# cule/multimot_track

Hardware: AMD Instinct MI355X
Metric: KITTI RGB-D frames/sec (ego+object poses) at 1/2/4/8 GPUs; CPU ref fps (higher is better)
Workload: dtype u8

## Files before the change

### include/mmt.h

```cpp
#ifndef MMT_H
#define MMT_H

#include <stddef.h>
#include <stdint.h>

#ifdef __cplusplus
extern "C" {
#endif

#define MMT_OK 0
#define MMT_EINVAL (-22)
#define MMT_ENOMEM (-12)
#define MMT_ENOSPC (-28)
#define MMT_EDEVICE (-5)
#define MMT_ESTATE (-77)

#define MMT_MAX_OBJECTS 15

typedef struct mmt_config {
  int width, height;
  float fx, fy, cx, cy;
  float k1, k2, p1, p2, k3;
  float bf;
  float th_depth;
// ... 75 lines not shown
                   const float* flow_uv, const int32_t* mask, double timestamp,
                   mmt_frame_result* res, mmt_motion* objs, int objs_cap);

int mmt_track_rgbd_chunk(mmt_ctx* ctx, int nframes, const uint8_t* const* bgr,
                         const uint16_t* const* disp256, const float* const* flow_uv,
                         const int32_t* const* mask, mmt_frame_result* res, mmt_motion* objs,
                         int objs_cap);

void* mmt_host_alloc(mmt_ctx* ctx, size_t bytes);
void mmt_host_free(mmt_ctx* ctx, void* p);

int mmt_track_rgbd_chunk_device(mmt_ctx* ctx, int nframes, const uint8_t* d_bgr,
                                size_t bgr_pitch, const uint16_t* d_disp, size_t disp_pitch,
                                const float* d_flow, size_t flow_pitch, const int32_t* d_mask,
                                size_t mask_pitch, mmt_frame_result* res, mmt_motion* objs,
                                int objs_cap, void* stream);

typedef struct mmt_flow_problem {
  int n;
  const float* obs;
  const float* flow;
  const float* depth;
  float Tcw_last[16];
  float init[16];
  float rp_thres;
  double prior_info;
  int max_iters;
  int use_noise;
  float g0;
  float fx, fy, cx, cy;
} mmt_flow_problem;
int mmt_pose_flow_solve(mmt_ctx* ctx, const mmt_flow_problem* problem, float* pose_out,
                        int* stats_out );

typedef struct mmt_pose_opt_problem {
  int n;
  const float* Xw;
  const float* obs;
  const float* inv_sigma2;
  float Tcw[16];
  float fx, fy, cx, cy, bf;
} mmt_pose_opt_problem;
int mmt_pose_optimization(mmt_ctx* ctx, const mmt_pose_opt_problem* problem, float* pose_out,
                          uint8_t* outlier_out, int* n_inliers);

int mmt_pnp_ransac(mmt_ctx* ctx, const float* pts3, const float* pts2, int n, float fx,
                   float fy, float cx, float cy, int max_iters, double reproj, double confidence,
                   double* R_out, double* t_out, int* inliers_out, int* n_inliers,
                   int* iters_out );

typedef struct mmt_pnpsolver_problem {
  int n;
  const float* pts3;
  const float* pts2;
  const float* sigma2;
  float fx, fy, cx, cy;
  double probability;
  int min_inliers;
  int max_iterations;
  int min_set;
  float epsilon;
  float th2;
} mmt_pnpsolver_problem;

typedef struct mmt_pnpsolver_state {
  int iterations;
// ... 303 lines not shown
```

### multimot_track_amd/__init__.py

```python
import ctypes
import os

import numpy as np

_HERE = os.path.dirname(os.path.abspath(__file__))
LIB_PATH = os.environ.get("MMT_LIB_PATH") or os.path.join(_HERE, "libmmt.so")
_LIB = None

KP_DTYPE = np.dtype([("x", "<f4"), ("y", "<f4"), ("size", "<f4"), ("angle", "<f4"),
                     ("response", "<f4"), ("octave", "<i4"), ("class_id", "<i4")])


class MmtConfig(ctypes.Structure):
    _fields_ = [("width", ctypes.c_int), ("height", ctypes.c_int),
                ("fx", ctypes.c_float), ("fy", ctypes.c_float), ("cx", ctypes.c_float),
                ("cy", ctypes.c_float), ("k1", ctypes.c_float), ("k2", ctypes.c_float),
                ("p1", ctypes.c_float), ("p2", ctypes.c_float), ("k3", ctypes.c_float),
                ("bf", ctypes.c_float), ("th_depth", ctypes.c_float), ("rgb", ctypes.c_int),
                ("orb_nfeatures", ctypes.c_int), ("orb_scale_factor", ctypes.c_float),
                ("orb_nlevels", ctypes.c_int), ("orb_ini_th_fast", ctypes.c_int),
                ("orb_min_th_fast", ctypes.c_int), ("noise_seed", ctypes.c_uint32),
                ("device_id", ctypes.c_int), ("max_batch", ctypes.c_int),
                ("fps", ctypes.c_float)]

# ... 497 lines not shown
            flow.data_ptr(), pitch(flow), mask.data_ptr(), pitch(mask), res, objs, MAX_OBJECTS,
            ctypes.c_void_p(stream)))
        if not parse:
            return res, objs
        return [_frame_dict(res[i], objs[i * MAX_OBJECTS:(i + 1) * MAX_OBJECTS])
                for i in range(nf)]

    def profile_enable(self, on=True):
        self._check(lib().mmt_profile_enable(self._h, int(on)))

    def profile_read(self, reset=False):
        p = MmtProfile()
        self._check(lib().mmt_profile_read(self._h, ctypes.byref(p), int(reset)))
        return dict(orb_ms=p.orb_ms, orb_launches=p.orb_launches, orb_frames=p.orb_frames)

    def flow_solve(self, obs, flow, depth, tcw_last, init, rp_thres, prior_info, max_iters,
                   K, use_noise=False, g0=0.0):
        obs = np.ascontiguousarray(obs, np.float32)
        flow = np.ascontiguousarray(flow, np.float32)
        depth = np.ascontiguousarray(depth, np.float32)
        pr = MmtFlowProblem()
        pr.n = len(depth)
        pr.obs, pr.flow, pr.depth = obs.ctypes.data, flow.ctypes.data, depth.ctypes.data
        pr.Tcw_last[:] = np.asarray(tcw_last, np.float32).reshape(16).tolist()
        pr.init[:] = np.asarray(init, np.float32).reshape(16).tolist()
        pr.rp_thres, pr.prior_info, pr.max_iters = rp_thres, prior_info, max_iters
        pr.use_noise, pr.g0 = int(use_noise), g0
        pr.fx, pr.fy, pr.cx, pr.cy = K
        pose = np.zeros(16, np.float32)
        st = np.zeros(3, np.int32)
        self._check(lib().mmt_pose_flow_solve(self._h, ctypes.byref(pr), _p(pose), _p(st)))
        return int(st[2]), pose.reshape(4, 4), dict(iterations=int(st[0]), inliers=int(st[1]))

    def pose_optimization(self, Xw, obs, inv_sigma2, tcw, K, bf):
        Xw = np.ascontiguousarray(Xw, np.float32)
        obs = np.ascontiguousarray(obs, np.float32)
        s2 = np.ascontiguousarray(inv_sigma2, np.float32)
        n = len(Xw)
        pr = MmtPoseOptProblem()
        pr.n = n
        pr.Xw, pr.obs, pr.inv_sigma2 = Xw.ctypes.data, obs.ctypes.data, s2.ctypes.data
        pr.Tcw[:] = np.asarray(tcw, np.float32).reshape(16).tolist()
        pr.fx, pr.fy, pr.cx, pr.cy = K
        pr.bf = bf
        pose = np.zeros(16, np.float32)
        out = np.zeros(max(n, 1), np.uint8)
        ninl = ctypes.c_int(0)
        self._check(lib().mmt_pose_optimization(self._h, ctypes.byref(pr), _p(pose), _p(out),
                                                ctypes.byref(ninl)))
        return ninl.value, pose.reshape(4, 4), out[:n].astype(bool)

    @staticmethod
    def _match_frame(kps, desc, depth, tcw, keep):
        kps = np.ascontiguousarray(kps)
        desc = np.ascontiguousarray(desc, np.uint8) if desc is not None else None
        depth = np.ascontiguousarray(depth, np.float32)
        keep += [kps, desc, depth]
        fr = MmtMatchFrame()
        fr.n = len(kps)
        fr.kps = kps.ctypes.data
        fr.desc = desc.ctypes.data if desc is not None else None
        fr.depth = depth.ctypes.data
        fr.Tcw[:] = np.asarray(tcw, np.float32).reshape(16).tolist()
        return fr

    def frame_grid(self, kps, depth):
# ... 481 lines not shown
```

### multimot_track_amd/csrc/mmt_capi_probes.hip

```cpp

#include <hip/hip_runtime.h>

#include <cstdint>

#include <algorithm>
#include <cmath>
#include <cstring>
#include <vector>

#include "mmt_ctx.h"
#include "mmt_devbuf.h"
#include "mmt_mat4.h"
#include "mmt_match.h"
#include "mmt_pnp.h"
#include "mmt_sim3.h"
#include "mmt_sim3opt.h"
#include "mmt_track.h"

using mmt::ArgError;
using mmt::DevBuf;
using mmt::DeviceError;

struct ProbeStage : mmt::Stage {
  uint8_t* d = nullptr;
// ... 101 lines not shown

static void check_feature_vector(const mmt_feature_vector* v, int n, std::vector<uint8_t>* once,
                                 int max_node) {
  if (v->n_nodes < 0) throw ArgError("negative node count");
  if (v->n_nodes == 0) return;
  if (!v->node_id || !v->node_start || !v->feat) throw ArgError("null feature vector arrays");
  if (v->node_start[0] != 0) throw ArgError("node_start[0] != 0");
  for (int k = 0; k < v->n_nodes; k++) {
    if (k > 0 && !(v->node_id[k - 1] < v->node_id[k])) throw ArgError("node ids not ascending");
    const int a = v->node_start[k], b = v->node_start[k + 1];
    if (b < a) throw ArgError("node_start not monotone");
    if (b - a > max_node) throw ArgError("a vocabulary node holds more than 16384 frame features");
    for (int q = a; q < b; q++) {
      const int f = v->feat[q];
      if (f < 0 || f >= n) throw ArgError("feature index out of range");
      if (once) {
        if ((*once)[f]) throw ArgError("a frame feature is listed in two nodes");
        (*once)[f] = 1;
      }
    }
  }
}

static void check_sft_keyframe(const mmt_sft_keyframe* k) {
  if (k->n < 0 || k->n > mmt::kMaxMatchKeys) throw ArgError("bad keyframe size");
  if (k->n > 0 && (!k->kps || !k->desc || !k->uR || !k->has_mp))
    throw ArgError("null keyframe arrays");
  std::vector<uint8_t> once((size_t)std::max(k->n, 1), 0);
  check_feature_vector(&k->fv, k->n, &once, INT32_MAX);
}

extern "C" {

int mmt_pose_flow_solve(mmt_ctx* ctx, const mmt_flow_problem* pr, float* pose_out,
                        int* stats_out) {
  if (!ctx || !pr || !pose_out || !stats_out || pr->n < 0) return MMT_EINVAL;
  return guard(ctx, [&] {
    MMT_HIP(hipSetDevice(ctx->cfg.device_id));
    hipStream_t s = ctx->stream;
    const int n = pr->n, cap = std::max(n, 1);
    DevBuf<float2> obs(cap), flow(cap);
    DevBuf<float> depth(cap), pose(16);
    DevBuf<double> scratch(mmt::flow_scratch_doubles(cap));
    DevBuf<int> st(3);
    DevBuf<mmt::FlowSolveDesc> dd(1);
    const int groups = mmt::flow_split_groups(n);
    DevBuf<unsigned long long> gx(groups > 1 ? mmt::kFlowSplitGranules : 1);
    if (groups > 1)
      MMT_HIP(hipMemsetAsync(gx.p, 0, sizeof(unsigned long long) * mmt::kFlowSplitGranules, s));
    obs.up((const float2*)pr->obs, n, s);
    flow.up((const float2*)pr->flow, n, s);
    depth.up(pr->depth, n, s);
    mmt::FlowSolveDesc d;
    memset(&d, 0, sizeof(d));
    d.n = n;
    d.obs = obs.p;
    d.flow = flow.p;
    d.depth = depth.p;
    memcpy(d.Tcw_last, pr->Tcw_last, 64);
    memcpy(d.init, pr->init, 64);
    d.rp_thres = pr->rp_thres;
    d.use_noise = pr->use_noise;
    d.g0 = pr->g0;
    d.max_iters = pr->max_iters;
    d.prior_info = pr->prior_info;
    d.fx = pr->fx; d.fy = pr->fy; d.cx = pr->cx; d.cy = pr->cy;
    d.scratch = scratch.p;
    d.cap = cap;
    d.pose_out = pose.p;
    d.stats = st.p;
    d.gx = gx.p;
    d.gx_seq = 1;
    dd.up(&d, 1, s);
    pose.up(pr->init, 16, s);
    if (groups > 1)
      mmt::launch_flow_lm_split(dd.p, groups, s);
    else
      mmt::launch_flow_lm(dd.p, 1, n, s);
    pose.down(pose_out, 16, s);
    st.down(stats_out, 3, s);
    MMT_HIP(hipStreamSynchronize(s));
    if (stats_out[2] == 2)
      throw mmt::DeviceError("pose flow solve: the split solve's workgroups were not resident together");
  });
}

int mmt_pose_optimization(mmt_ctx* ctx, const mmt_pose_opt_problem* pr, float* pose_out,
                          uint8_t* outlier_out, int* n_inliers) {
  if (!ctx || !pr || !pose_out || !n_inliers || pr->n < 0 ||
      (pr->n > 0 && (!pr->Xw || !pr->obs || !pr->inv_sigma2 || !outlier_out)))
    return MMT_EINVAL;
  return guard(ctx, [&] {
    MMT_HIP(hipSetDevice(ctx->cfg.device_id));
    hipStream_t s = ctx->stream;
    const int n = pr->n, cap = std::max(n, 1);
    DevBuf<float> X(3 * (size_t)cap), ob(3 * (size_t)cap), s2(cap), pose(16);
    DevBuf<uint8_t> outl(cap);
    DevBuf<int> ninl(1), fsc(n > mmt::kPoseOptMaxEdges ? cap : 1);
    DevBuf<double> esc(n > mmt::kPoseOptMaxEdges ? 3 * (size_t)cap : 1);
    DevBuf<mmt::PoseOptDesc> dd(1);
    X.up(pr->Xw, 3 * (size_t)n, s);
    ob.up(pr->obs, 3 * (size_t)n, s);
    s2.up(pr->inv_sigma2, n, s);
    mmt::PoseOptDesc d;
    memset(&d, 0, sizeof(d));
    d.n = n;
    d.Xw = X.p;
    d.obs = ob.p;
    d.inv_sigma2 = s2.p;
    memcpy(d.Tcw, pr->Tcw, 64);
    d.fx = pr->fx; d.fy = pr->fy; d.cx = pr->cx; d.cy = pr->cy; d.bf = pr->bf;
    d.pose_out = pose.p;
    d.outlier = outl.p;
    d.n_inliers = ninl.p;
    d.e_scratch = esc.p;
    d.f_scratch = fsc.p;
    dd.up(&d, 1, s);
// ... 571 lines not shown
```

### multimot_track_amd/csrc/mmt_lm.hip

```cpp

#include <hip/hip_runtime.h>

#include <cfloat>
#include <cstdio>
#include <cstdlib>

#include <algorithm>

#include "mmt_devmath.h"
#include "mmt_internal.h"
#include "mmt_lmstep.h"
#include "mmt_track.h"

namespace mmt {

namespace {

constexpr double kInfo = 0.1;

struct LMItem {
  double X[3];
  double ob[2];
  double pr[2];
  double f[2];
// ... 579 lines not shown
#pragma unroll
    for (int cc = 0; cc < 3; cc++) Rwl[3 * r + cc] = D.Tcw_last[4 * cc + r];
#pragma unroll
  for (int r = 0; r < 3; r++) {
    double s = 0;
#pragma unroll
    for (int k = 0; k < 3; k++) s += (double)Rwl[3 * r + k] * (double)D.Tcw_last[4 * k + 3];
    twl[r] = (float)(-s);
  }
  auto init_item = [&](int i, LMItem& it) {
    const int s = D.idx ? D.idx[i] : i;
    const float2 ob = D.obs[s];
    float z = D.depth[s];
    if (D.use_noise) z = (float)((double)z + (double)D.g0 * ((double)(z * z) / (725 * 0.5) * 0.15));
    const double u = ob.x, v = ob.y, dz = z;
    const double Xc0 = (u - c.cx) * dz / c.fx, Xc1 = (v - c.cy) * dz / c.fy, Xc2 = dz;
    it.X[0] = (double)Rwl[0] * Xc0 + (double)Rwl[1] * Xc1 + (double)Rwl[2] * Xc2 + (double)twl[0];
    it.X[1] = (double)Rwl[3] * Xc0 + (double)Rwl[4] * Xc1 + (double)Rwl[5] * Xc2 + (double)twl[1];
    it.X[2] = (double)Rwl[6] * Xc0 + (double)Rwl[7] * Xc1 + (double)Rwl[8] * Xc2 + (double)twl[2];
    it.ob[0] = u;
    it.ob[1] = v;
    const float2 fl = D.flow[s];
    it.pr[0] = fl.x;
    it.pr[1] = fl.y;
    it.f[0] = fl.x;
    it.f[1] = fl.y;
    it.xl[0] = it.xl[1] = 0;
    it.e[0] = it.e[1] = 0;
  };
  LMItem R[IR];
  const int n_reg = IR * nt;
  constexpr bool kCacheB = true;
  double RB[12];
  DSE3 P = dse3_from_float(D.init);
  const double hin = kInfo + c.pinfo;
  double* row = tile_row(sm.tile);
  {
    double mh = 0;
#pragma unroll
    for (int k = 0; k < IR; k++) {
      const int i = tid + k * nt;
      if (i < N) {
        init_item(lo + i, R[k]);
        if (k == 0)
          linearise<true>(c, P, R[k], R[k].f[0], R[k].f[1], row, 0.0, R[k].e[0], R[k].e[1],
                          R[k].w, R[k].bl[0], R[k].bl[1], mh, kCacheB ? RB : nullptr);
        else
          linearise<false>(c, P, R[k], R[k].f[0], R[k].f[1], row, 0.0, R[k].e[0], R[k].e[1],
                           R[k].w, R[k].bl[0], R[k].bl[1], mh);
      }
    }
    for (int i = n_reg + tid; i < N; i += nt) {
      LMItem it;
      init_item(lo + i, it);
      linearise<false>(c, P, it, it.f[0], it.f[1], row, 0.0, it.e[0], it.e[1], it.w, it.bl[0],
                       it.bl[1], mh);
      item_store(G, cap, lo + i, it);
    }
    if (tid >= N)
      for (int q = 0; q < kSums; q++) row[q] = 0;
#pragma unroll
    for (int o = 32; o > 0; o >>= 1) mh = fmax(mh, __shfl_xor(mh, o, 64));
    if ((tid & 63) == 0) sm.mh[tid >> 6] = mh;
  }
  int pb = 0;
  double vc = block_sum_tile_lanes<kSums>(sm.tile, sm.part[pb], nw);
  pb ^= 1;
// ... 1047 lines not shown
```

### multimot_track_amd/csrc/mmt_map.h

```cpp
#pragma once
#include <hip/hip_runtime.h>

#include <cstdint>
#include <functional>
#include <set>
#include <utility>
#include <vector>

#include "mmt_ba.h"
#include "mmt_bow.h"
#include "mmt_internal.h"
#include "mmt_mapgraph.h"
#include "mmt_match.h"
#include "mmt_track.h"

namespace mmt {

struct MapCamH {
  int W = 0, H = 0;
  float fx = 0, fy = 0, cx = 0, cy = 0, invfx = 0, invfy = 0, bf = 0;
  float thDepth = 0;
  int maxFrames = 0;
  int nlevels = 0;
  float logScale = 0;
// ... 22 lines not shown
  long n_lm = 0;
};

struct BowStatsH {
  long n_bow_frames = 0, n_trk = 0, n_trk_ok = 0, n_reloc = 0, n_reloc_ok = 0, n_reloc_cands = 0,
       n_pnp_found = 0, n_sbp_rounds = 0, n_triangulated = 0, n_sft_matches = 0, n_kfdb = 0;
};

struct MapStatsH {
  int state = 0;
  int matches_mm = -1;
  int inliers_local = -1;
  int n_keyframes = 0, n_mappoints = 0;
  int new_keyframe = 0;
  float Tcw_map[16];
};

constexpr size_t kDescBytes = 256;
constexpr size_t kOutHdr = 128;

class MapEngine {
 public:
  ~MapEngine();
  void setup(const MapCamH& cam, int kcap);
  void reset();
  long next_frame_id() { return frameNextId_++; }
  void prepare(MapFrameH& F) const;
  void initialize(MapFrameH& C, const float* Tcw);
  int track(MapFrameH& C, const GridFrame& G, float* Tcw, MapFrameH& L, float* Tlast, float* vel,
            bool& has_vel, bool& bSecondFrame, MapStatsH& st, hipStream_t s);
  void track_finish(MapFrameH& C, MapFrameH& L, const float* Tcw, MapStatsH& st);
  void set_overlap(std::function<void()> fn) { overlap_ = std::move(fn); }
  bool overlap_pending() const { return (bool)overlap_; }
  void frame_done(const MapFrameH& C, const float* Tcw);
  int state() const { return state_; }
  int n_keyframes() const { return graph_.n_keyframes(); }
  int n_mappoints() const { return graph_.n_mappoints(); }
  void set_frame_grid(const GridFrame& G) { G_ = G; }
  const MappingStats& mapping_stats() const { return mstats_; }
  void blk_time(int k, double& t) {
    if (!prof_on_) return;
    const double n = now_us();
    mstats_.blk_us[k] += n - t;
    t = n;
  }
  void set_cull_ratio(double r) { cull_ratio_ = r; }
  void dump(int32_t* sizes, const mmt_map_dump_arrays* out) const { graph_.dump(sizes, out); }
  void set_vocabulary(Vocabulary* v);
  const BowStatsH& bow_stats() const { return bstats_; }

 private:
  std::function<void()> overlap_;
  MapGraph graph_;
  LocalPointCache lpc_;
  std::vector<FuseKF> kf_dev_;
  std::vector<int> kf_count_, kf_touched_;
  bool spec_on_ = true, spec_valid_ = false;
  bool overlap_c3_ = true;
  long spec_frame_ = -1, spec_stamp_ = 0, spec_hits_ = 0, spec_tries_ = 0;
  std::vector<int> spec_mps_, spec_cnt_, spec_touched_, spec_kfs_, spec_pts_;
  std::vector<long> spec_mark_;
  uint8_t* h_early_ = nullptr;
  hipEvent_t ev_early_ = nullptr;
  void speculate_local_map(const MapFrameH& L, int n);
  bool commit_local_map(MapFrameH& C);
  void spec_discard();
  void collect_checked(const std::vector<int>& kfl, std::vector<int>& out, long& gen);
  long ids_uploads_ = 0;
  long local_gen_ = 0, spec_gen_ = 0;
  void run_overlap() {
    if (!overlap_) return;
    std::function<void()> fn = std::move(overlap_);
    overlap_ = nullptr;
    fn();
  }
  static constexpr int kTemp = MapGraph::kTemp;
  bool track_with_motion_model(MapFrameH& C, const GridFrame& G, float* Tcw, MapFrameH& L,
                               float* Tlast, const float* vel, MapStatsH& st);
  bool track_reference_subst(MapFrameH& C, const GridFrame& G, float* Tcw, const MapFrameH& L,
                             const float* Tlast);
  bool relocalization_subst(MapFrameH& C, const GridFrame& G, float* Tcw, const float* Tlast,
                            const float* vel);
  bool track_local_map(MapFrameH& C, const GridFrame& G, float* Tcw);
  int discard_outliers(MapFrameH& C, int nmatches, int* nmatchesMap);
  void update_last_frame(MapFrameH& L, float* Tlast);
  void update_local_keyframes(MapFrameH& C);
  void update_local_points();
  void search_local_points(MapFrameH& C, const GridFrame& G, const float* Tcw);
  bool need_new_keyframe(const MapFrameH& C);
  void create_new_keyframe(MapFrameH& C, const float* Tcw);
  void process_new_keyframe(int kf);
  void map_point_culling(int kf);
  void local_mapping(int kf);
  void search_in_neighbors(int kf);
  void fuse_sequence(const std::vector<int>& kfl, const std::vector<int>& pts);
  void fuse_apply(int kf, int h, int bestIdx, int bestDist);
  void local_bundle_adjustment(int kf);
  void keyframe_culling(int kf);
  void kf_set_bad(int kf);
  void kf_store_add(int kf);
  void bow_launch(const uint8_t* d_desc, int n, hipStream_t st);
  void bow_finish(int n, hipStream_t st, BowVecH& v, FeatVecH& fv);
// ... 135 lines not shown
```

### multimot_track_amd/csrc/mmt_map.hip

```cpp

#include <hip/hip_runtime.h>

#include <algorithm>
#include <climits>
#include <cstdio>
#include <cstdlib>
#include <cmath>
#include <cstring>

#include "mmt_map.h"
#include "mmt_mat4.h"

namespace mmt {

#define MAP_PROF(k, stmt)                       \
  do {                                          \
    const double _t0 = prof_on_ ? now_us() : 0; \
    stmt;                                       \
    if (prof_on_) prof_[k] += now_us() - _t0;   \
  } while (0)

MapEngine::~MapEngine() {
  if (prof_on_ && prof_n_ > 0) {
    static const char* names[12] = {"C2 search", "D1 (motion model)", "local map update",
                                    "C3 search", "D1 (local map)", "keyframe + mapping",
                                    "other", "total", "UpdateLastFrame", "C2 pack",
                                    "C3 pack", "D1 pack"};
    fprintf(stderr, "[mmt map profile] %ld frames, host wall us per frame:", prof_n_);
    for (int k = 0; k < 12; k++) fprintf(stderr, " %s %.1f%s", names[k], prof_[k] / prof_n_,
                                         k < 11 ? "," : "\n");
    if (mstats_.n_lm > 0) {
      const double n = (double)mstats_.n_lm;
      fprintf(stderr, "[mmt localmapping profile] %ld keyframes, host wall us per keyframe: "
              "ProcessNewKeyFrame+MapPointCulling %.1f, CreateNewMapPoints + SearchInNeighbors %.1f "
              "(CreateNewMapPoints %.1f, Fuse launches "
              "%.1f), LocalBundleAdjustment %.1f (solve %.1f), KeyFrameCulling %.1f, final sync "
              "%.1f, LocalMapping total %.1f; CreateNewKeyFrame with all of it %.1f\n", mstats_.n_lm,
              mstats_.pnk_us / n,
              mstats_.sin_us / n, mstats_.cnmp_us / n, mstats_.fuse_us / n, mstats_.ba_us / n,
              mstats_.basolve_us / n, mstats_.cull_us / n, mstats_.lmsync_us / n,
              mstats_.lm_us / n, mstats_.kfnew_us / n);
      static const char* bn[MappingStats::kBlk] = {
          "new keyframe + store", "new points", "SIN targets", "SIN fuse 1", "SIN candidates",
          "SIN fuse 2", "SIN point updates", "SIN connections", "BA graph", "BA apply",
          "Fuse pool flush", "Fuse enqueue", "Fuse wait", "Fuse apply (+ relaunches)",
          "ComputeDistinctiveDescriptors (inside the others)", "PNK ComputeBoW",
          "PNK observations", "PNK UpdateConnections"};
      fprintf(stderr, "[mmt localmapping profile] per keyframe, us:");
      for (int k = 0; k < MappingStats::kBlk; k++)
        fprintf(stderr, " %s %.1f%s", bn[k],
                (k == 14 ? graph_.stats().distinctive_us : mstats_.blk_us[k]) / n,
                k + 1 < MappingStats::kBlk ? "," : "\n");
    }
    fprintf(stderr, "[mmt map profile] per frame: %.1f local keyframes, %.1f local points, "
            "%.1f C3 edges; %zu map points allocated, %d keyframes at the end; local map "
            "speculated %ld times, taken %ld; local point list cache (MMT_LOCALMAP_CACHE=%d) "
            "hits %ld, rebuilds %ld (%ld of them after a structure edit, %ld ids uploads)\n",
            prof_cnt_[0] / prof_n_, prof_cnt_[1] / prof_n_, prof_cnt_[2] / prof_n_, graph_.n_points(),
            n_keyframes(), spec_tries_, spec_hits_, lpc_.mode(), lpc_.hits(), lpc_.rebuilds(),
            lpc_.epoch_rebuilds(), ids_uploads_);
  }
  if (s_) (void)hipStreamSynchronize(s_);
  if (lm_s_) {
    (void)hipStreamSynchronize(lm_s_);
    (void)hipStreamDestroy(lm_s_);
  }
  if (ev_early_) (void)hipEventDestroy(ev_early_);
  for (void* p : dallocs_) (void)hipFree(p);
  for (void* p : hallocs_) (void)hipHostFree(p);
}

static size_t last_bytes(int n) { return (size_t)n * (sizeof(mmt_kp) + 12 + 32 + 2); }

static_assert(sizeof(PoseOptDesc) <= kDescBytes, "PoseOptDesc outgrew its slot");
static size_t align16(size_t x) { return (x + 15) & ~(size_t)15; }

struct SelLayout {
  size_t ids, skip, taken, bX, bHas, total;
  SelLayout(int m, int n, bool ids_inline = true) {
    ids = kDescBytes;
    skip = ids + (ids_inline ? 4 * (size_t)m : 0);
    taken = skip + m;
    bX = align16(taken + n);
    bHas = bX + 12 * (size_t)n;
    total = bHas + n;
  }
};

size_t MapEngine::out_bytes(int n) const { return kOutHdr + 4 * (size_t)kcap_ + n; }

void MapEngine::setup(const MapCamH& cam, int kcap) {
  cam_ = cam;
  kcap_ = kcap;
  d_last_ = dev<uint8_t>(kDescBytes + last_bytes(kcap));
  h_last_ = pinned<uint8_t>(kDescBytes + last_bytes(kcap));
  c2_ = CandSet{dev<uint32_t>((size_t)kcap * kCandK), dev<int>((size_t)kcap * kCandK),
                dev<int>(kcap), dev<PointWin>(kcap), dev<int>(kcap)};
  d_out_ = dev<uint8_t>(kOutHdr + 5 * (size_t)kcap);
  h_out_ = pinned<uint8_t>(kOutHdr + 5 * (size_t)kcap);
  d_nm_ = (int*)d_out_;
  d_ninl_ = (int*)(d_out_ + 4);
  d_pose_ = (float*)(d_out_ + 16);
  d_match_ = (int*)(d_out_ + kOutHdr);
  d_outl_ = d_out_ + kOutHdr + 4 * (size_t)kcap;
  h_nm_ = (int*)h_out_;
  h_ninl_ = (int*)(h_out_ + 4);
  h_pose_ = (float*)(h_out_ + 16);
  h_match_ = (int*)(h_out_ + kOutHdr);
  h_outl_ = h_out_ + kOutHdr + 4 * (size_t)kcap;
  d_edges_ = dev<float>(7 * (size_t)kcap);
  h_edges_ = pinned<float>(7 * (size_t)kcap);
  d_esc_ = dev<double>(3 * (size_t)kcap);
  d_fsc_ = dev<int>(kcap);
  prof_on_ = getenv("MMT_MAP_PROFILE") != nullptr;
  if (const char* e = getenv("MMT_LOCALMAP_SPEC")) spec_on_ = atoi(e) != 0;
  if (const char* e = getenv("MMT_OVERLAP_C3")) overlap_c3_ = atoi(e) != 0;
  int lpc_mode = 1, lpc_ways = 4;
  if (const char* e = getenv("MMT_LOCALMAP_CACHE")) lpc_mode = atoi(e);
  if (const char* e = getenv("MMT_LOCALMAP_CACHE_WAYS")) lpc_ways = atoi(e);
  lpc_ = LocalPointCache(lpc_mode, lpc_ways);
  graph_.setup(cam_.scale, cam_.nlevels, prof_on_);
  h_early_ = pinned<uint8_t>(kOutHdr + 4 * (size_t)kcap);
  MMT_HIP(hipEventCreateWithFlags(&ev_early_, hipEventDisableTiming));
  int prio_lo = 0, prio_hi = 0;
  MMT_HIP(hipDeviceGetStreamPriorityRange(&prio_lo, &prio_hi));
  const char* lmp = getenv("MMT_LM_PRIO");
  const int lm_prio = lmp && strcmp(lmp, "high") == 0 ? prio_hi : 0;
  MMT_HIP(hipStreamCreateWithPriority(&lm_s_, hipStreamNonBlocking, lm_prio));
  kf_rec_bytes_ = align16(sizeof(mmt_kp) * (size_t)kcap) + 32 * (size_t)kcap +
                  align16(4 * (size_t)kcap) + align16(4 * (size_t)(kGridCells + 1)) +
                  align16(4 * (size_t)kcap);
  frameNextId_ = 0;
  mbVO_ = false;
  matchesInliers_ = 0;
  lastRelocFrameId_ = 0;
  reset();
}

void MapEngine::grow_local(int m) {
  if (m <= local_cap_ && d_sel_) return;
  const int cap = std::max(m + 4096, 2 * local_cap_);
  void* old[] = {d_sel_, h_sel_, d_inview_, h_inview_, c3_.key, c3_.idx, c3_.n, c3_.win,
                 c3_.choice, d_ids_, h_ids_};
  if (s_) MMT_HIP(hipStreamSynchronize(s_));
  for (int i = 0; i < 11; i++) {
    if (!old[i]) continue;
    const bool host = i == 1 || i == 3 || i == 10;
    auto it = std::find(host ? hallocs_.begin() : dallocs_.begin(),
                        host ? hallocs_.end() : dallocs_.end(), old[i]);
    if (host) {
      (void)hipHostFree(old[i]);
      hallocs_.erase(it);
    } else {
      (void)hipFree(old[i]);
      dallocs_.erase(it);
    }
// ... 588 lines not shown
  float* bX = (float*)(h_sel_ + sl.bX);
  uint8_t* bHas = h_sel_ + sl.bHas;
  int nbase = 0;
  for (int i = 0; i < C.n; i++) {
    const int h = C.mps[i];
    taken[i] = 0;
    bHas[i] = h >= 0;
    if (h >= 0) {
      const MPoint& p = graph_.mp(h);
      taken[i] = p.nObs() > 0;
      memcpy(bX + 3 * (size_t)i, p.pos, 12);
      nbase++;
    }
  }
  if (prof_on_) prof_[10] += now_us() - t_pack;
  pose_desc_fill(h_sel_, d_sel_, Tcw);
  MMT_HIP(hipMemcpyAsync(d_sel_, h_sel_, sl.total, hipMemcpyHostToDevice, s_));
  if (!ids_inline && ids_new) {
    if (m > 0) MMT_HIP(hipMemcpyAsync(d_ids_, h_ids_, 4 * (size_t)m, hipMemcpyHostToDevice, s_));
    ids_gen_ = local_gen_;
  }
  const float th = curId_ < lastRelocFrameId_ + 2 ? 5.f : 3.f;
  LocalSel sel{d_ids, d_sel_ + sl.skip, d_inview_};
  MapEdgeArgs e = edge_args(G);
  e.pool = d_pool_;
  e.ids = d_ids;
  e.has_base = d_sel_ + sl.bHas;
  e.base_X = (const float*)(d_sel_ + sl.bX);
  launch_search_local(G, Tcw, d_pool_, d_pool_desc_, m, th, d_sel_ + sl.taken, nullptr, c3_,
                      d_match_, d_nm_, s_, &sel, &e);
  launch_pose_opt(d_pod_, 1, std::min(C.n, nbase + m), s_);
  MMT_HIP(hipMemcpyAsync(h_out_, d_out_, out_bytes(C.n), hipMemcpyDeviceToHost, s_));
  if (m > 0) MMT_HIP(hipMemcpyAsync(h_inview_, d_inview_, (size_t)m, hipMemcpyDeviceToHost, s_));
  run_overlap();
  MMT_HIP(hipStreamSynchronize(s_));
  for (int j = 0; j < m; j++)
    if (!skip[j] && h_inview_[j]) graph_.mp(localPts_[j]).visible++;
  for (int i = 0; i < C.n; i++)
    if (h_match_[i] >= 0) C.mps[i] = localPts_[h_match_[i]];
}

bool MapEngine::track_local_map(MapFrameH& C, const GridFrame& G, float* Tcw) {
  MAP_PROF(2, if (!commit_local_map(C)) {
    update_local_keyframes(C);
    update_local_points();
  });
  if (prof_on_) {
    prof_cnt_[0] += localKFs_.size();
    prof_cnt_[1] += localPts_.size();
  }
  MAP_PROF(3, search_local_points(C, G, Tcw));
  MAP_PROF(4, apply_pose_opt(C, Tcw));
  matchesInliers_ = 0;
  for (int i = 0; i < C.n; i++) {
    if (C.mps[i] < 0 || C.outlier[i]) continue;
    MPoint& p = graph_.mp(C.mps[i]);
    p.found++;
    if (p.nObs() > 0) matchesInliers_++;
  }
  if (curId_ < lastRelocFrameId_ + cam_.maxFrames && matchesInliers_ < 50) return false;
  return matchesInliers_ >= 30;
}

bool MapEngine::need_new_keyframe(const MapFrameH& C) {
  const int nKFs = n_keyframes();
  if (curId_ < lastRelocFrameId_ + cam_.maxFrames && nKFs > cam_.maxFrames) return false;
  const int nMinObs = nKFs <= 2 ? 2 : 3;
  const int nRefMatches = graph_.tracked_map_points(refKF_, nMinObs);
// ... 181 lines not shown
```

### multimot_track_amd/csrc/mmt_track.h

```cpp
#pragma once
#include <hip/hip_runtime.h>

#include <cstdint>

#include "../../include/mmt.h"

namespace mmt {

constexpr int kMaxLabel = 16;

struct SampleSet {
  float2* keys;
  float2* corres;
  float2* flow;
  float* depth;
  int* count;
  int cap;
};

struct ObjSampleSet {
  float2* keys;
  float2* corres;
  float2* flow;
  float* depth;
// ... 31 lines not shown
  float fx, fy, cx, cy;
  int W, H;
  int32_t* obj_label;
  int* members;
  int member_cap;
  LabelStats* stats;
  int* hist;
  int* err;
};

struct FlowSolveDesc {
  const int* d_n;
  int n;
  const int* idx;
  const float2* obs;
  const float2* flow;
  const float* depth;
  float Tcw_last[16];
  float init[16];
  float rp_thres;
  int use_noise;
  float g0;
  int max_iters;
  double prior_info;
  float fx, fy, cx, cy;
  double* scratch;
  int cap;
  float* pose_out;
  int* stats;
  float* centre_out;
  unsigned long long* gx;
  unsigned gx_seq;
  unsigned long long gx_spin;
};

constexpr int kFlowSplitMax = 8;
constexpr int kFlowSplitGranules = 2 * kFlowSplitMax * 128;
int flow_split_groups(int n_hint);
void launch_flow_lm_split(const FlowSolveDesc* d_desc, int groups, hipStream_t st);

void launch_gray_depth(const uint8_t* bgr, size_t bgr_pitch, const uint16_t* disp,
                       size_t disp_pitch, uint8_t* gray, size_t gray_pitch, float* depth,
                       size_t depth_pitch, int npix, int nframes, float bf, hipStream_t st);
void launch_static_samples(const mmt_kp* kps, const int* nkp, const float* depth,
                           const float2* flow, const int32_t* mask, int W, int H,
                           const SampleSet& out, hipStream_t st);
void launch_obj_samples(const float* depth, const float2* flow, const int32_t* mask, int W,
                        int H, const ObjSampleSet& out, hipStream_t st);
void launch_handoff(const float2* last_corres, const int* n_last, const float2* last_ocorres,
                    const int* n_olast, const float* depth, const int32_t* mask, int W, int H,
                    const HandoffSet& cur, hipStream_t st);
void launch_obj_group(const GroupArgs& a, hipStream_t st);
void launch_flow_lm(const FlowSolveDesc* d_descs, int nsolves, int n_hint, hipStream_t st);
size_t flow_scratch_doubles(int cap);

struct PoseOptDesc {
  int n;
  const float* Xw;
  const float* obs;
  const float* inv_sigma2;
  float Tcw[16];
  double fx, fy, cx, cy, bf;
  float* pose_out;
  uint8_t* outlier;
  int* n_inliers;
  double* e_scratch;
// ... 7 lines not shown
```

### multimot_track_amd/csrc/mmt_tracker.h

```cpp
#pragma once
#include <hip/hip_runtime.h>

#include <cstdint>
#include <deque>
#include <string>
#include <vector>

#include "mmt_internal.h"
#include "mmt_map.h"
#include "mmt_pnp.h"
#include "mmt_track.h"

namespace mmt {

constexpr int kMaxObj = kMaxLabel - 1;
constexpr int kRansacIters = 500;

struct ObjOut {
  int label = 0, sem_label = 0, n_points = 0, n_ransac_inliers = 0, n_mm_inliers = -1;
  int ransac_iterations = 0, n_solve = 0, n_inliers = 0, iterations = 0;
  float init[16], X[16], motion[16];
  float centre_pre[3] = {0, 0, 0};
};

// ... 65 lines not shown
    std::vector<std::vector<float>> vObjMod;
  };
  struct ObjFrame {
    bool active = false;
    bool a_launched = false;
    int cur = 0, last = 0, slot = 0, nobj = 0;
    FrameOut* out = nullptr;
    std::vector<int> labels, LabId, PreObjID, members;
    PnPObject* po = nullptr;
  };
  struct FrameArgs {
    const float* depth;
    const float2* flow;
    const int32_t* mask;
    const mmt_kp* kps;
    const int* nkp;
    int n_keys;
    int f;
    int buf;
  };
  struct PnPBuf {
    float* pts3;
    float2* pts2;
    int* inliers;
    int* mm_inliers;
    int* subset;
    int* n_subset;
    int* result;
    double* Rt;
  };
  template <typename T>
  T* alloc(size_t n);
  void ego_launch(const FrameArgs& a, FrameOut& out, hipStream_t st);
  void ego_map_finish(FrameOut& out);
  void ego_finish(FrameOut& out, hipStream_t st);
  void obj_stage_a(ObjFrame& F);
  void obj_stage_a_launch(ObjFrame& F);
  void obj_stage_a_decide(ObjFrame& F);
  void obj_stage_b(ObjFrame& F);
  void obj_finish(ObjFrame& F);
  void obj_advance();
  void obj_flush();

  mmt_config cfg_{};
  OrbEngine* engine_ = nullptr;
  MapEngine map_;
  GridFrame grid0_{};
  float* d_uR_ = nullptr;
  float* d_kdepth_ = nullptr;
  int* d_cell_start_ = nullptr;
  int* d_cell_idx_ = nullptr;
  struct HostChunk {
    mmt_kp* kps = nullptr;
    uint8_t* desc = nullptr;
    float* uR = nullptr;
    float* kdepth = nullptr;
    int* nkp = nullptr;
    B3HostOut dev;
  };
  HostChunk hc_[2];
  int chunk_buf_ = 0;
  bool reset_pending_ = false;
  int W_ = 0, H_ = 0, max_chunk_ = 0, kcap_ = 0, ocap_ = 0, lm_cap_ = 0, mask_words_ = 0;
  float g0_ = 0;
  int state_ = 0, cur_ = 0, last_ = 2;
  bool bFirstFrame_ = false, bSecondFrame_ = false, hasVelocity_ = false;
  float V_[16] = {0};
  static constexpr int kSlots = 22;
  static constexpr int kObjSlots = 18;
  static constexpr int kObjLagMax = kObjSlots - 2;
  int obj_lag_ = 16;
  int d3_iters_ = 200;
  FrameSlot slot_[kSlots];
  struct EgoHost {
    FlowSolveDesc d2;
    float Tcw[16];
    int st[3];
    int nlast_obj;
    int n_static[3];
  };
  bool ego_pending_ = false;
  float ego_Tinit_[16];
  EgoHost* eh_ = nullptr;
  ObjFrame qa_;
  bool defer_ = false;
  long frame_seq_ = 0;
  std::deque<FrameOut> dq_;
  void deliver_deferred(std::vector<FrameOut>& outs, bool all);
  std::deque<ObjFrame> inflight_;
  int obj_slot_next_ = 0;
  struct ObjResults {
    int res[8 * kMaxObj];
    float init[16 * kMaxObj];
    float X[16 * kMaxObj];
    int lst[3 * kMaxObj];
    int nsub[kMaxObj];
    float centre[3 * kMaxObj];
  };
  struct ObjHost {
    LabelStats stats[kMaxLabel];
    int hist[kMaxLabel * kMaxLabel];
    int err;
    PnPObject po[kMaxObj];
    int subsets[kMaxObj][5 * kRansacIters];
    FlowSolveDesc descs[kMaxObj];
    ObjResults r;
  };
  static constexpr size_t kObjStatsBytes = sizeof(LabelStats) * kMaxLabel + sizeof(int) * kMaxLabel * kMaxLabel;
  static constexpr size_t kObjPnpBytes = sizeof(PnPObject) * kMaxObj + sizeof(int) * kMaxObj * 5 * kRansacIters;
  ObjHost* oh_[kObjSlots] = {};
  ObjResults* d_r_[kObjSlots] = {};
  double* d_Rt_[kObjSlots] = {};
  FlowSolveDesc* d_descs3_[kObjSlots] = {};
  hipEvent_t ev_ransac_[kObjSlots] = {};
// ... 52 lines not shown
```

### multimot_track_amd/csrc/mmt_tracker.hip

```cpp

#include <hip/hip_runtime.h>

#include <algorithm>
#include <cfloat>
#include <cmath>
#include <cstring>
#include <map>
#include <chrono>
#include <cstdio>
#include <cstdlib>
#include <vector>

#include "mmt_internal.h"
#include "mmt_map.h"
#include "mmt_mat4.h"
#include "mmt_pnp.h"
#include "mmt_track.h"
#include "mmt_tracker.h"

namespace mmt {

static inline uint64_t rng_next(uint64_t x) { return (uint64_t)(unsigned)x * 4164903690ULL + (x >> 32); }
float rng_first_gaussian(uint64_t seed) {
  static unsigned kn[128];
// ... 266 lines not shown
    mc.W = W_;
    mc.H = H_;
    mc.fx = cfg.fx; mc.fy = cfg.fy; mc.cx = cfg.cx; mc.cy = cfg.cy; mc.bf = cfg.bf;
    mc.invfx = 1.0f / cfg.fx;
    mc.invfy = 1.0f / cfg.fy;
    mc.thDepth = cfg.bf * cfg.th_depth / cfg.fx;
    mc.maxFrames = (int)(cfg.fps == 0.f ? 30.f : cfg.fps);
    mc.nlevels = t.nlevels;
    mc.scale = t.scale;
    mc.invSigma2 = t.invSigma2;
    mc.logScale = (float)std::log((double)t.scale[t.nlevels > 1 ? 1 : 0]);
    map_.setup(mc, kcap_);
    GridFrame& G = grid0_;
    memset(&G, 0, sizeof(G));
    G.fx = cfg.fx; G.fy = cfg.fy; G.cx = cfg.cx; G.cy = cfg.cy; G.bf = cfg.bf;
    G.minX = 0.0f; G.maxX = (float)W_; G.minY = 0.0f; G.maxY = (float)H_;
    G.invW = static_cast<float>(kGridCols) / static_cast<float>(G.maxX - G.minX);
    G.invH = static_cast<float>(kGridRows) / static_cast<float>(G.maxY - G.minY);
    G.nlevels = t.nlevels;
    for (int l = 0; l < t.nlevels; l++) G.scale[l] = t.scale[l];
    G.logScale = mc.logScale;
  }
  int lo = 0, hi = 0;
  MMT_HIP(hipDeviceGetStreamPriorityRange(&lo, &hi));
  (void)hi;
  MMT_HIP(hipStreamCreateWithPriority(&oa_, hipStreamNonBlocking, lo));
  MMT_HIP(hipStreamCreateWithPriority(&ob_, hipStreamNonBlocking, lo));
  MMT_HIP(hipHostMalloc((void**)&eh_, sizeof(EgoHost), hipHostMallocDefault));
  memset(eh_, 0, sizeof(EgoHost));
  reset();
  device_ = cfg.device_id;
  static_assert(kSlots > kObjLagMax + 2, "frame slots too few for the object lag");
  if (const char* ss = getenv("MMT_DEBUG_SPLIT_SPIN")) split_spin_ = strtoull(ss, nullptr, 10);
}

void Tracker::reset() {
  if (oa_) MMT_HIP(hipStreamSynchronize(oa_));
  if (ob_) MMT_HIP(hipStreamSynchronize(ob_));
  if (d_err_) MMT_HIP(hipMemset(d_err_, 0, sizeof(int)));
  state_ = 0;
  bFirstFrame_ = false;
  bSecondFrame_ = false;
  hasVelocity_ = false;
  cur_ = 0;
  last_ = kSlots - 1;
  ego_pending_ = false;
  qa_ = ObjFrame();
  inflight_.clear();
  obj_slot_next_ = 0;
  dq_.clear();
  frame_seq_ = 0;
  for (FrameSlot& F : slot_) {
    F.nModLabel.clear();
    F.nSemPosition.clear();
    F.vObjMod.clear();
    F.bSecond = false;
    F.obj_slot = -1;
    mat4_eye(F.Tcw);
    mat4_eye(F.Tview);
    F.m = MapFrameH();
  }
  map_.reset();
  reset_pending_ = false;
}

void Tracker::track_chunk(const uint8_t* d_bgr, size_t bgr_pitch, const uint16_t* d_disp,
// ... 196 lines not shown
    m.kps = hc.kps + (size_t)kcap_ * a.f;
    m.desc = hc.desc + 32 * (size_t)kcap_ * a.f;
    m.uR = hc.uR + (size_t)kcap_ * a.f;
    m.depth = hc.kdepth + (size_t)kcap_ * a.f;
    map_.prepare(m);
  }
  C.nModLabel.clear();
  C.nSemPosition.clear();
  C.vObjMod.clear();
  launch_static_samples(a.kps, a.nkp, a.depth, a.flow, a.mask, W_, H_, C.st, st);
  MMT_HIP(hipMemcpyAsync(&eh_->n_static[cur_], C.st.count, sizeof(int), hipMemcpyDeviceToHost, st));
  launch_obj_samples(a.depth, a.flow, a.mask, W_, H_, C.ob, st);
  const bool handoff = bFirstFrame_ || bSecondFrame_;
  if (handoff)
    launch_handoff(Ls.st.corres, Ls.st.count, Ls.ob.corres, Ls.ob.count, a.depth, a.mask, W_, H_,
                   C.ho, st);
  MMT_HIP(hipMemcpyAsync(&eh_->nlast_obj, handoff ? Ls.ob.count : C.ob.count, sizeof(int),
                         hipMemcpyDeviceToHost, st));
  GridFrame G = grid0_;
  G.keys = a.kps;
  G.desc = d_desc_ + 32 * (size_t)kcap_ * a.f;
  G.uR = d_uR_ + (size_t)kcap_ * a.f;
  G.cell_start = d_cell_start_ + (size_t)(kGridCells + 1) * a.f;
  G.cell_idx = d_cell_idx_ + (size_t)kcap_ * a.f;
  G.n = a.n_keys;
  map_.set_frame_grid(G);
  if (state_ == 0) {
    ego_pending_ = false;
    return;
  }
  {
    MapStatsH& ms = out.map;
    map_.set_overlap([this] { obj_advance(); });
    const int rr = map_.track(C.m, G, ego_Tinit_, Ls.m, Ls.Tview, V_, hasVelocity_,
                              bSecondFrame_, ms, st);
    map_.set_overlap(nullptr);
    ms.state = map_.state();
    memcpy(ms.Tcw_map, ego_Tinit_, sizeof(ego_Tinit_));
    if (rr == 1) {
      ms.n_keyframes = map_.n_keyframes();
      ms.n_mappoints = map_.n_mappoints();
      reset_pending_ = true;
      ego_pending_ = false;
      return;
    }
    map_finish_pending_ = true;
  }
  C.bSecond = bSecondFrame_;
  FlowSolveDesc& d2 = eh_->d2;
  memset(&d2, 0, sizeof(d2));
  d2.d_n = Ls.st.count;
  d2.idx = nullptr;
  d2.obs = Ls.st.keys;
  d2.flow = Ls.st.flow;
  d2.depth = Ls.st.depth;
  memcpy(d2.Tcw_last, Ls.Tview, sizeof(d2.Tcw_last));
  memcpy(d2.init, ego_Tinit_, sizeof(d2.init));
  d2.rp_thres = 0.04f;
  d2.use_noise = 1;
  d2.g0 = g0_;
  d2.max_iters = 100;
  d2.prior_info = 0.3;
  d2.fx = cfg_.fx; d2.fy = cfg_.fy; d2.cx = cfg_.cx; d2.cy = cfg_.cy;
  d2.scratch = d_lm_scratch_;
  d2.cap = lm_cap_;
  d2.pose_out = d_poses_;
  d2.stats = d_lmstats_;
  d2.gx = d_gx_;
  d2.gx_seq = ++gx_seq_;
  d2.gx_spin = split_spin_;
  if ((gx_seq_ & 0xFFFFu) == 0)
    MMT_HIP(hipMemsetAsync(d_gx_, 0, sizeof(unsigned long long) * kFlowSplitGranules, st));
  MMT_HIP(hipMemcpyAsync(d_descs_, &d2, sizeof(d2), hipMemcpyHostToDevice, st));
  const int groups = flow_split_groups(eh_->n_static[last_]);
  if (groups > 1)
    launch_flow_lm_split(d_descs_, groups, st);
  else
    launch_flow_lm(d_descs_, 1, eh_->n_static[last_], st);
  MMT_HIP(hipMemcpyAsync(eh_->Tcw, d_poses_, sizeof(eh_->Tcw) + sizeof(eh_->st),
                         hipMemcpyDeviceToHost, st));
  ego_pending_ = true;
}

void Tracker::ego_map_finish(FrameOut& out) {
  if (!map_finish_pending_) return;
  map_finish_pending_ = false;
  FrameSlot& C = slot_[cur_];
  FrameSlot& Ls = slot_[last_];
  map_.track_finish(C.m, Ls.m, ego_Tinit_, out.map);
  out.map.n_keyframes = map_.n_keyframes();
  out.map.n_mappoints = map_.n_mappoints();
}

void Tracker::ego_finish(FrameOut& out, hipStream_t st) {
  FrameSlot& C = slot_[cur_];
  FrameSlot& Ls = slot_[last_];
  MMT_HIP(hipStreamSynchronize(st));
  if (defer_) {
    dq_.emplace_back();
    dq_.back().seq = out.seq;
  }
  out.n_obj_samples = eh_->nlast_obj;
  bool advance = true;
  if (reset_pending_) {
    memcpy(out.Tcw, ego_Tinit_, sizeof(out.Tcw));
    out.initialized = false;
    return;
  }
  if (state_ == 0) {
    bFirstFrame_ = true;
    bSecondFrame_ = false;
    if (out.n_keys > 500) {
      mat4_eye(C.Tcw);
      memcpy(C.Tview, C.Tcw, sizeof(C.Tview));
// ... 454 lines not shown
```

Baseline: 743.7.

## Chain ego flow solve on device after map pose optimization

Enqueues the ego flow Levenberg-Marquardt solve right after the map pose-optimization kernel, reading its initial pose from device memory (new init_dev field). This removes a host round trip before that launch. The map tracker now waits on an event instead of synchronizing the whole stream. If the host-side final pose differs from the device pose used, the solve is synchronized and re-enqueued; this adds a redo path and relies on cross-stream ordering between the map stream and the ego stream.

```diff
diff --git a/include/mmt.h b/include/mmt.h
--- a/include/mmt.h
+++ b/include/mmt.h
@@ -131,6 +131,9 @@
 } mmt_flow_problem;
 int mmt_pose_flow_solve(mmt_ctx* ctx, const mmt_flow_problem* problem, float* pose_out,
                         int* stats_out );
+int mmt_pose_flow_solve_init_dev(mmt_ctx* ctx, const mmt_flow_problem* problem,
+                                 int init_on_device, float* pose_out, int* stats_out,
+                                 float* centre_out);
 
 typedef struct mmt_pose_opt_problem {
   int n;
diff --git a/multimot_track_amd/__init__.py b/multimot_track_amd/__init__.py
--- a/multimot_track_amd/__init__.py
+++ b/multimot_track_amd/__init__.py
@@ -553,6 +553,30 @@
         self._check(lib().mmt_pose_flow_solve(self._h, ctypes.byref(pr), _p(pose), _p(st)))
         return int(st[2]), pose.reshape(4, 4), dict(iterations=int(st[0]), inliers=int(st[1]))
 
+    def flow_solve_init_dev(self, obs, flow, depth, tcw_last, init, rp_thres, prior_info,
+                            max_iters, K, init_on_device, use_noise=False, g0=0.0):
+        obs = np.ascontiguousarray(obs, np.float32)
+        flow = np.ascontiguousarray(flow, np.float32)
+        depth = np.ascontiguousarray(depth, np.float32)
+        pr = MmtFlowProblem()
+        pr.n = len(depth)
+        pr.obs, pr.flow, pr.depth = obs.ctypes.data, flow.ctypes.data, depth.ctypes.data
+        pr.Tcw_last[:] = np.asarray(tcw_last, np.float32).reshape(16).tolist()
+        pr.init[:] = np.asarray(init, np.float32).reshape(16).tolist()
+        pr.rp_thres, pr.prior_info, pr.max_iters = rp_thres, prior_info, max_iters
+        pr.use_noise, pr.g0 = int(use_noise), g0
+        pr.fx, pr.fy, pr.cx, pr.cy = K
+        pose = np.zeros(16, np.float32)
+        st = np.zeros(3, np.int32)
+        centre = np.zeros(3, np.float32)
+        fn = lib().mmt_pose_flow_solve_init_dev
+        fn.argtypes = [ctypes.c_void_p, ctypes.POINTER(MmtFlowProblem), ctypes.c_int32,
+                       ctypes.c_void_p, ctypes.c_void_p, ctypes.c_void_p]
+        self._check(fn(self._h, ctypes.byref(pr), int(init_on_device), _p(pose), _p(st),
+                       _p(centre)))
+        return (int(st[2]), pose.reshape(4, 4), dict(iterations=int(st[0]), inliers=int(st[1])),
+                centre)
+
     def pose_optimization(self, Xw, obs, inv_sigma2, tcw, K, bf):
         Xw = np.ascontiguousarray(Xw, np.float32)
         obs = np.ascontiguousarray(obs, np.float32)
diff --git a/multimot_track_amd/csrc/mmt_capi_probes.hip b/multimot_track_amd/csrc/mmt_capi_probes.hip
--- a/multimot_track_amd/csrc/mmt_capi_probes.hip
+++ b/multimot_track_amd/csrc/mmt_capi_probes.hip
@@ -157,15 +157,15 @@
 
 extern "C" {
 
-int mmt_pose_flow_solve(mmt_ctx* ctx, const mmt_flow_problem* pr, float* pose_out,
-                        int* stats_out) {
+static int flow_solve_probe(mmt_ctx* ctx, const mmt_flow_problem* pr, bool init_on_device,
+                            float* pose_out, int* stats_out, float* centre_out) {
   if (!ctx || !pr || !pose_out || !stats_out || pr->n < 0) return MMT_EINVAL;
   return guard(ctx, [&] {
     MMT_HIP(hipSetDevice(ctx->cfg.device_id));
     hipStream_t s = ctx->stream;
     const int n = pr->n, cap = std::max(n, 1);
     DevBuf<float2> obs(cap), flow(cap);
-    DevBuf<float> depth(cap), pose(16);
+    DevBuf<float> depth(cap), pose(16), init(16), centre(3);
     DevBuf<double> scratch(mmt::flow_scratch_doubles(cap));
     DevBuf<int> st(3);
     DevBuf<mmt::FlowSolveDesc> dd(1);
@@ -196,6 +196,12 @@
     d.stats = st.p;
     d.gx = gx.p;
     d.gx_seq = 1;
+    if (centre_out) d.centre_out = centre.p;
+    if (init_on_device) {
+      init.up(pr->init, 16, s);
+      d.init_dev = init.p;
+      memset(d.init, 0xFF, sizeof(d.init));
+    }
     dd.up(&d, 1, s);
     pose.up(pr->init, 16, s);
     if (groups > 1)
@@ -204,10 +210,21 @@
       mmt::launch_flow_lm(dd.p, 1, n, s);
     pose.down(pose_out, 16, s);
     st.down(stats_out, 3, s);
+    if (centre_out) centre.down(centre_out, 3, s);
     MMT_HIP(hipStreamSynchronize(s));
     if (stats_out[2] == 2)
       throw mmt::DeviceError("pose flow solve: the split solve's workgroups were not resident together");
   });
+}
+
+int mmt_pose_flow_solve(mmt_ctx* ctx, const mmt_flow_problem* pr, float* pose_out,
+                        int* stats_out) {
+  return flow_solve_probe(ctx, pr, false, pose_out, stats_out, nullptr);
+}
+
+int mmt_pose_flow_solve_init_dev(mmt_ctx* ctx, const mmt_flow_problem* pr, int init_on_device,
+                                 float* pose_out, int* stats_out, float* centre_out) {
+  return flow_solve_probe(ctx, pr, init_on_device != 0, pose_out, stats_out, centre_out);
 }
 
 int mmt_pose_optimization(mmt_ctx* ctx, const mmt_pose_opt_problem* pr, float* pose_out,
diff --git a/multimot_track_amd/csrc/mmt_lm.hip b/multimot_track_amd/csrc/mmt_lm.hip
--- a/multimot_track_amd/csrc/mmt_lm.hip
+++ b/multimot_track_amd/csrc/mmt_lm.hip
@@ -635,7 +635,7 @@
   const int n_reg = IR * nt;
   constexpr bool kCacheB = true;
   double RB[12];
-  DSE3 P = dse3_from_float(D.init);
+  DSE3 P = dse3_from_float(D.init_dev ? D.init_dev : D.init);
   const double hin = kInfo + c.pinfo;
   double* row = tile_row(sm.tile);
   {
diff --git a/multimot_track_amd/csrc/mmt_map.h b/multimot_track_amd/csrc/mmt_map.h
--- a/multimot_track_amd/csrc/mmt_map.h
+++ b/multimot_track_amd/csrc/mmt_map.h
@@ -78,6 +78,10 @@
   void track_finish(MapFrameH& C, MapFrameH& L, const float* Tcw, MapStatsH& st);
   void set_overlap(std::function<void()> fn) { overlap_ = std::move(fn); }
   bool overlap_pending() const { return (bool)overlap_; }
+  void set_after_d1(std::function<void(const float*)> fn) { after_d1_ = std::move(fn); }
+  void count_d2(int kind) { d2_count_[kind]++; }
+  void set_d2_chain_mode(int m) { d2_chain_mode_ = m; }
+  const float* d1_pose_host() const { return h_pose_; }
   void frame_done(const MapFrameH& C, const float* Tcw);
   int state() const { return state_; }
   int n_keyframes() const { return graph_.n_keyframes(); }
@@ -114,6 +118,10 @@
   void collect_checked(const std::vector<int>& kfl, std::vector<int>& out, long& gen);
   long ids_uploads_ = 0;
   long local_gen_ = 0, spec_gen_ = 0;
+  std::function<void(const float*)> after_d1_;
+  hipEvent_t ev_d1_ = nullptr;
+  long d2_count_[3] = {0, 0, 0};
+  int d2_chain_mode_ = 1;
   void run_overlap() {
     if (!overlap_) return;
     std::function<void()> fn = std::move(overlap_);
diff --git a/multimot_track_amd/csrc/mmt_map.hip b/multimot_track_amd/csrc/mmt_map.hip
--- a/multimot_track_amd/csrc/mmt_map.hip
+++ b/multimot_track_amd/csrc/mmt_map.hip
@@ -55,10 +55,12 @@
     fprintf(stderr, "[mmt map profile] per frame: %.1f local keyframes, %.1f local points, "
             "%.1f C3 edges; %zu map points allocated, %d keyframes at the end; local map "
             "speculated %ld times, taken %ld; local point list cache (MMT_LOCALMAP_CACHE=%d) "
-            "hits %ld, rebuilds %ld (%ld of them after a structure edit, %ld ids uploads)\n",
+            "hits %ld, rebuilds %ld (%ld of them after a structure edit, %ld ids uploads); flow "
+            "solves (MMT_D2_CHAIN=%d) chained %ld, host-launched %ld, redone %ld\n",
             prof_cnt_[0] / prof_n_, prof_cnt_[1] / prof_n_, prof_cnt_[2] / prof_n_, graph_.n_points(),
             n_keyframes(), spec_tries_, spec_hits_, lpc_.mode(), lpc_.hits(), lpc_.rebuilds(),
-            lpc_.epoch_rebuilds(), ids_uploads_);
+            lpc_.epoch_rebuilds(), ids_uploads_, d2_chain_mode_, d2_count_[0], d2_count_[1],
+            d2_count_[2]);
   }
   if (s_) (void)hipStreamSynchronize(s_);
   if (lm_s_) {
@@ -66,6 +68,7 @@
     (void)hipStreamDestroy(lm_s_);
   }
   if (ev_early_) (void)hipEventDestroy(ev_early_);
+  if (ev_d1_) (void)hipEventDestroy(ev_d1_);
   for (void* p : dallocs_) (void)hipFree(p);
   for (void* p : hallocs_) (void)hipHostFree(p);
 }
@@ -122,6 +125,7 @@
   graph_.setup(cam_.scale, cam_.nlevels, prof_on_);
   h_early_ = pinned<uint8_t>(kOutHdr + 4 * (size_t)kcap);
   MMT_HIP(hipEventCreateWithFlags(&ev_early_, hipEventDisableTiming));
+  MMT_HIP(hipEventCreateWithFlags(&ev_d1_, hipEventDisableTiming));
   int prio_lo = 0, prio_hi = 0;
   MMT_HIP(hipDeviceGetStreamPriorityRange(&prio_lo, &prio_hi));
   const char* lmp = getenv("MMT_LM_PRIO");
@@ -776,8 +780,15 @@
   launch_pose_opt(d_pod_, 1, std::min(C.n, nbase + m), s_);
   MMT_HIP(hipMemcpyAsync(h_out_, d_out_, out_bytes(C.n), hipMemcpyDeviceToHost, s_));
   if (m > 0) MMT_HIP(hipMemcpyAsync(h_inview_, d_inview_, (size_t)m, hipMemcpyDeviceToHost, s_));
+  if (after_d1_) {
+    MMT_HIP(hipEventRecord(ev_d1_, s_));
+    after_d1_(d_pose_);
+  }
   run_overlap();
-  MMT_HIP(hipStreamSynchronize(s_));
+  if (after_d1_)
+    MMT_HIP(hipEventSynchronize(ev_d1_));
+  else
+    MMT_HIP(hipStreamSynchronize(s_));
   for (int j = 0; j < m; j++)
     if (!skip[j] && h_inview_[j]) graph_.mp(localPts_[j]).visible++;
   for (int i = 0; i < C.n; i++)
diff --git a/multimot_track_amd/csrc/mmt_track.h b/multimot_track_amd/csrc/mmt_track.h
--- a/multimot_track_amd/csrc/mmt_track.h
+++ b/multimot_track_amd/csrc/mmt_track.h
@@ -87,6 +87,7 @@
   unsigned long long* gx;
   unsigned gx_seq;
   unsigned long long gx_spin;
+  const float* init_dev;
 };
 
 constexpr int kFlowSplitMax = 8;
diff --git a/multimot_track_amd/csrc/mmt_tracker.h b/multimot_track_amd/csrc/mmt_tracker.h
--- a/multimot_track_amd/csrc/mmt_tracker.h
+++ b/multimot_track_amd/csrc/mmt_tracker.h
@@ -121,6 +121,7 @@
   template <typename T>
   T* alloc(size_t n);
   void ego_launch(const FrameArgs& a, FrameOut& out, hipStream_t st);
+  void enqueue_d2(const float* init_dev, hipStream_t st);
   void ego_map_finish(FrameOut& out);
   void ego_finish(FrameOut& out, hipStream_t st);
   void obj_stage_a(ObjFrame& F);
@@ -169,6 +170,9 @@
     int n_static[3];
   };
   bool ego_pending_ = false;
+  bool d2_chain_ = true;
+  bool d2_queued_ = false;
+  hipStream_t ego_st_ = nullptr;
   float ego_Tinit_[16];
   EgoHost* eh_ = nullptr;
   ObjFrame qa_;
diff --git a/multimot_track_amd/csrc/mmt_tracker.hip b/multimot_track_amd/csrc/mmt_tracker.hip
--- a/multimot_track_amd/csrc/mmt_tracker.hip
+++ b/multimot_track_amd/csrc/mmt_tracker.hip
@@ -322,6 +322,13 @@
   device_ = cfg.device_id;
   static_assert(kSlots > kObjLagMax + 2, "frame slots too few for the object lag");
   if (const char* ss = getenv("MMT_DEBUG_SPLIT_SPIN")) split_spin_ = strtoull(ss, nullptr, 10);
+  if (const char* e = getenv("MMT_D2_CHAIN")) d2_chain_ = atoi(e) != 0;
+  map_.set_d2_chain_mode(d2_chain_ ? 1 : 0);
+  if (d2_chain_)
+    map_.set_after_d1([this](const float* d_pose) {
+      enqueue_d2(d_pose, ego_st_);
+      d2_queued_ = true;
+    });
 }
 
 void Tracker::reset() {
@@ -584,6 +591,8 @@
   {
     MapStatsH& ms = out.map;
     map_.set_overlap([this] { obj_advance(); });
+    ego_st_ = st;
+    d2_queued_ = false;
     const int rr = map_.track(C.m, G, ego_Tinit_, Ls.m, Ls.Tview, V_, hasVelocity_,
                               bSecondFrame_, ms, st);
     map_.set_overlap(nullptr);
@@ -599,6 +608,22 @@
     map_finish_pending_ = true;
   }
   C.bSecond = bSecondFrame_;
+  if (d2_queued_ && memcmp(ego_Tinit_, map_.d1_pose_host(), sizeof(ego_Tinit_)) == 0) {
+    map_.count_d2(0);
+  } else {
+    if (d2_queued_) {
+      MMT_HIP(hipStreamSynchronize(st));
+      map_.count_d2(2);
+    } else {
+      map_.count_d2(1);
+    }
+    enqueue_d2(nullptr, st);
+  }
+  ego_pending_ = true;
+}
+
+void Tracker::enqueue_d2(const float* init_dev, hipStream_t st) {
+  FrameSlot& Ls = slot_[last_];
   FlowSolveDesc& d2 = eh_->d2;
   memset(&d2, 0, sizeof(d2));
   d2.d_n = Ls.st.count;
@@ -607,7 +632,10 @@
   d2.flow = Ls.st.flow;
   d2.depth = Ls.st.depth;
   memcpy(d2.Tcw_last, Ls.Tview, sizeof(d2.Tcw_last));
-  memcpy(d2.init, ego_Tinit_, sizeof(d2.init));
+  if (init_dev)
+    d2.init_dev = init_dev;
+  else
+    memcpy(d2.init, ego_Tinit_, sizeof(d2.init));
   d2.rp_thres = 0.04f;
   d2.use_noise = 1;
   d2.g0 = g0_;
@@ -631,7 +659,6 @@
     launch_flow_lm(d_descs_, 1, eh_->n_static[last_], st);
   MMT_HIP(hipMemcpyAsync(eh_->Tcw, d_poses_, sizeof(eh_->Tcw) + sizeof(eh_->st),
                          hipMemcpyDeviceToHost, st));
-  ego_pending_ = true;
 }
 
 void Tracker::ego_map_finish(FrameOut& out) {
```

New measurement: 770.1 (median of 6 runs). 1.04x the previous value.
